# zcash/halo2

Hardware: NVIDIA H100
Metric: msm_pairs_per_s (higher is better)
Workload: dtype u32x8 (255-bit modular integers)

## Files before the change

halo2_b200/csrc/capi_msm.cu:

```cuda
#define H2_MSM_QUAD_ACCUM_REFS (g_ctx.small_accum_refs)
#include "util_kernels.cuh"
#include "msm.cuh"
#include "ipa.cuh"
#include "ntt.cuh"
#include "ecfft.cuh"
#include "fixedbase.cuh"
static_assert(H2_FB_BITS == H2_FB_BITS_CTX, "ctx.cuh: fixed_table");


static int exclusive_scan_u32(uint32_t *d, uint64_t n, cudaStream_t s, const uint32_t *only_if = nullptr) {
    const uint64_t per_block = (uint64_t)H2_SCAN_BLOCK * H2_SCAN_ITEMS;
    uint32_t nb = (uint32_t)((n + per_block - 1) / per_block);
    if (g_ctx.scan_blocks.ensure((size_t)nb * 4 + 16)) return 1;
    uint32_t *bs = g_ctx.scan_blocks.as<uint32_t>();
    LAUNCH(scan_block_sums_kernel, nb, H2_SCAN_BLOCK, 0, s, d, n, bs, only_if);
    LAUNCH(scan_single_block_kernel, 1, H2_SCAN_BLOCK, 0, s, bs, nb, only_if);
    LAUNCH(scan_apply_kernel, nb, H2_SCAN_BLOCK, 0, s, d, n, bs, only_if);
    return 0;
}

uint32_t g_chunk_cut[H2_MAX_UPLOAD_CHUNKS + 1][H2_MAX_UPLOAD_CHUNKS + 1] = {
    {0, 16, 16, 16, 16}, {0, 16, 16, 16, 16}, {0, 4, 16, 16, 16}, {0, 2, 8, 16, 16}, {0, 1, 4, 10, 16}};
static inline size_t chunk_first(size_t n, uint32_t k, uint32_t j) {
    const auto &cut = g_chunk_cut;
// ... 76 lines not shown
        FbPlan fp;
        fp.total = n; fp.sets = sets ? sets : 1u; fp.split = fb_split(n, fp.sets); fp.scalars_mont = scalars_mont ? 1u : 0u;
        record(2, H2_FB_BITS, H2_FB_WINDOWS, fp.sets, 2, 0, 0);
        const uint64_t count0 = n * fp.split;
        if (X.fb_a.ensure(fp.sets * count0 * sizeof(xyzz)) || X.fb_b.ensure(fp.sets * fb_ctas(count0, fb_fan(count0)) * sizeof(xyzz))) return 1;
        issue = [&X, fp, count0, d_scalars, d_bases, d_out, out_canonical, s]() -> int {
            auto k_acc = fb_accum_kernel<P, PS>;
            auto k_red = fb_reduce_kernel<P, PS>;
            xyzz *a = X.fb_a.as<xyzz>(), *b = X.fb_b.as<xyzz>();
            prof_begin(PROF_MSM_ACCUM0, s);
            LAUNCH(k_acc, blocks_for(fp.sets * count0, 128), 128, 0, s, fp, d_scalars, d_bases, a);
            prof_end(s);
            uint64_t count = count0, in_stride = count0;
            for (;;) {
                const uint32_t f = fb_fan(count);
                const uint64_t ctas = fb_ctas(count, f);
                LAUNCH(k_red, dim3((unsigned)ctas, fp.sets), 4 * H2_FB_QUADS, 0, s, (const xyzz *)a, count, in_stride, f, b, ctas,
                       ctas == 1 ? d_out : (jacobian *)nullptr, (uint32_t)out_canonical);
                if (ctas == 1) break;
                xyzz *t = a; a = b; b = t;
                count = ctas; in_stride = ctas;
            }
            return 0;
        };
        return msm_issue_or_replay(issue, !bc, d_scalars, d_bases, d_out, n, stride, H2_FB_BITS, fp.sets, scalars_mont, out_canonical, s);
    }
    const uint32_t glv = (!fixed && X.glv_on && n < (1ull << 30)) ? 1u : 0u;
    if (c == 0) c = X.window_override ? X.window_override : msm_default_window(n, glv);
    if (c > 24) return fail("msm: window bits > 24");
    const uint32_t K = (bc && !fixed && bc->k > 1) ? bc->k : 1u;
    const uint32_t force_cap = X.sort_bins ? 0u : H2_MSM_NO_BINS;
    MsmPlan p;
    msm_make_plan(p, n, c, 0, 0, fixed, stride, glv, sets, force_cap);
    p.chunks = K;
    p.fast = (fixed == 1 && !bc && X.fast_now && p.cap != 0) ? 1u : 0u;
    X.last_fast = p.fast != 0;
    if (p.fast && p.T < p.cap) { p.T = p.cap; p.acc_chunk[0] = p.T; }
    p.natural = (p.fast && p.G <= X.natural_max_buckets && p.max_refs <= 2 * H2_MSM_QUAD_ACCUM_REFS && (X.accum_ways <= 1 || X.accum_ways >= 12)) ? 1u : 0u;
    MsmPlan pk[H2_MAX_UPLOAD_CHUNKS];
    size_t first[H2_MAX_UPLOAD_CHUNKS + 1];
    for (uint32_t j = 0; j <= K; j++) first[j] = chunk_first(n, K, j);
    uint64_t ref_space = 0, max_items = 0, part_total = 0;
    uint32_t t_max = 0;
    for (uint32_t j = 0; j < K; j++) {
        if (K == 1) pk[0] = p;
        else msm_make_plan(pk[j], first[j + 1] - first[j], c, 0, 0, fixed, stride, glv, sets, force_cap);
        if (pk[j].ref_space >= (1ull << 32)) return fail("msm: n * windows exceeds 2^32 references");
        ref_space = pk[j].ref_space > ref_space ? pk[j].ref_space : ref_space;
        max_items = pk[j].max_items > max_items ? pk[j].max_items : max_items;
        part_total = pk[j].part_total > part_total ? pk[j].part_total : part_total;
        t_max = pk[j].T > t_max ? pk[j].T : t_max;
    }
    bool thread_per_item = false;
    for (uint32_t j = 0; j < K; j++) thread_per_item |= pk[j].max_refs > (pk[j].fixed ? 2 : 1) * H2_MSM_QUAD_ACCUM_REFS;
    record(fixed, c, p.W, p.sets, thread_per_item ? 1u : 0u, p.natural, p.fast);
    uint64_t ba_space = 0;
    if (!fixed && X.ba_rounds) {
        size_t free_b = 0, total_b = 0;
        CU(cudaMemGetInfo(&free_b, &total_b));
        for (uint32_t j = 0; j < K; j++) {
            if (pk[j].max_refs > H2_MSM_QUAD_ACCUM_REFS && (uint64_t)K * pk[j].ref_space * 56 <= free_b / 2) msm_plan_ba(pk[j], X.ba_rounds, X.ba_target);
            if (pk[j].ba) ba_space = pk[j].ref_space > ba_space ? pk[j].ref_space : ba_space;
        }
    }
    if (K == 1) p.ba = pk[0].ba;
    if (ba_space)
        for (uint32_t r = 0; r < H2_BA_MAX_ROUNDS; r++)
            if (X.ba_lv[r].ensure(K * ((ba_space >> (r + 1)) + 1) * sizeof(affine))) return 1;
    if (glv && (X.bases_phi.ensure(n * sizeof(affine)) || X.glv_parts.ensure(n * 32))) return 1;
    if (fixed && (uint64_t)p.W * stride >= (1ull << 31)) return fail("msm: window table too large for 31-bit references");
    if (p.G >= (1ull << 32) || n >= (1ull << 31)) return fail("msm: n * windows exceeds 2^32 references");
    if (scalars_mont && X.scal_canon.ensure(n * p.sets * sizeof(fe))) return 1;
    const size_t small_words = 2 * (t_max + 2) + 8;
    part_total += 1;
    if (X.counts.ensure(K * (p.G + 1) * 4) || X.cursor.ensure(K * 2 * p.G * 4) || X.refs.ensure(K * ref_space * 4) ||
        X.size_hist.ensure(K * small_words * 4) || X.items.ensure(K * max_items * sizeof(uint2)) ||
        X.bucket_sum.ensure(K * p.G * sizeof(xyzz)) || X.pkey.ensure(K * part_total * 4) || X.pstart.ensure(K * part_total * 4) ||
        X.pend.ensure(K * part_total * 4) || X.ppt.ensure(K * part_total * sizeof(xyzz)) ||
        X.ra_t.ensure((size_t)p.Wb * p.m1 * sizeof(xyzz)) || X.ra_e.ensure((size_t)p.Wb * p.m1 * sizeof(xyzz)) ||
        X.r0.ensure((size_t)p.Wb * p.nb0 * H2_R0_ROWS * sizeof(xyzz)) || X.r1.ensure((size_t)p.Wb * p.r1_rows * sizeof(xyzz)) ||
        X.wsum.ensure((size_t)p.Wb * sizeof(xyzz)))
        return 1;
    MsmBuffers Mk[H2_MAX_UPLOAD_CHUNKS];
    for (uint32_t j = 0; j < K; j++) {
        MsmBuffers &M = Mk[j];
        const size_t o = first[j];
        M.scalars = d_scalars + o; M.bases = d_bases + o; M.bases_phi = X.bases_phi.as<affine>() + o;
        M.glv_parts = X.glv_parts.as<uint32_t>() + 8 * o; M.scalars_mont = scalars_mont ? 1u : 0u;
        M.scal_canon = X.scal_canon.as<fe>() + o;
        M.counts = X.counts.as<uint32_t>() + j * (p.G + 1); M.cursor = X.cursor.as<uint32_t>() + j * 2 * p.G; M.cursor2 = M.cursor + p.G;
        M.refs = X.refs.as<uint32_t>() + j * ref_space;
        M.size_hist = X.size_hist.as<uint32_t>() + j * small_words; M.size_cursor = M.size_hist + (pk[j].T + 2); M.flags = M.size_cursor + (pk[j].T + 2);
        M.items = X.items.as<uint2>() + j * max_items;
        M.bucket_sum = X.bucket_sum.as<xyzz>() + j * p.G;
        for (uint32_t r = 0; r < H2_BA_MAX_ROUNDS; r++) M.ba[r] = ba_space ? X.ba_lv[r].as<affine>() + j * ((ba_space >> (r + 1)) + 1) : nullptr;
        M.pkey = X.pkey.as<uint32_t>() + j * part_total; M.pstart = X.pstart.as<uint32_t>() + j * part_total;
        M.pend = X.pend.as<uint32_t>() + j * part_total; M.ppt = X.ppt.as<xyzz>() + j * part_total;
        M.ra_t = X.ra_t.as<xyzz>(); M.ra_e = X.ra_e.as<xyzz>(); M.r0 = X.r0.as<xyzz>(); M.r1 = X.r1.as<xyzz>();
        M.wsum = X.wsum.as<xyzz>(); M.result = d_out;
    }
    X.last_flags = Mk[0].flags;

    {
        const uint64_t per_block = (uint64_t)H2_SCAN_BLOCK * H2_SCAN_ITEMS;
        if (X.scan_blocks.ensure((size_t)((p.G + 1 + per_block - 1) / per_block) * 4 + 16)) return 1;
    }
    issue = [&]() -> int {
        if (!p.fast) CU(cudaMemsetAsync(X.counts.p, 0, K * (p.G + 1) * 4, s));
        CU(cudaMemsetAsync(X.cursor.p, 0, K * 2 * p.G * 4, s));
        CU(cudaMemsetAsync(X.size_hist.p, 0, K * small_words * 4, s));
        CU(cudaMemsetAsync(X.bucket_sum.p, 0, K * p.G * sizeof(xyzz), s));
        if (!p.fast) CU(cudaMemsetAsync(X.pkey.p, 0xff, K * part_total * 4, s));

        auto k_bin = msm_bin_kernel<P, PS>;
        auto k_hist = msm_hist_kernel<P, PS>;
        auto k_scatter = msm_scatter_kernel<P, PS>;
        auto k_ihist = msm_item_hist_kernel<P, PS>;
        auto k_ibases = msm_item_bases_kernel<P, PS>;
        auto k_iplace = msm_item_place_kernel<P, PS>;
        auto k_accum0 = msm_accum0_kernel<P, PS>;
        auto k_accum0q = msm_accum0_quad_kernel<P, PS>;
        auto k_accum0p2 = msm_accum0_pair_kernel<P, PS>;
        auto k_accum0s2 = msm_accum0_split_kernel<P, PS, 2>;
        auto k_accum0s4 = msm_accum0_split_kernel<P, PS, 4>;
        auto k_accum0m2 = msm_accum0_multi_kernel<P, PS, 2>;
        auto k_accum0m4 = msm_accum0_multi_kernel<P, PS, 4>;
        auto k_ba = X.ba_variant == 1 ? msm_ba_round_kernel<P, PS, 4, 5> : X.ba_variant == 2 ? msm_ba_round_kernel<P, PS, 2, 4>
                  : X.ba_variant == 3 ? msm_ba_round_kernel<P, PS, 2, 5> : msm_ba_round_kernel<P, PS, 4, 4>;
        auto k_accum0p = msm_accum0_pts_kernel<P, PS>;
        auto k_accumN = msm_accumN_kernel<P, PS>;
        auto k_rest = msm_accum_rest_kernel<P, PS>;
        auto k_reduceA = msm_reduceA_kernel<P, PS>;
        auto k_r0 = msm_r0_kernel<P, PS>;
        auto k_r1 = msm_r1_kernel<P, PS>;
        auto k_wsum = msm_wsum_kernel<P, PS>;
        auto k_final = msm_final_kernel<P, PS>;
        for (uint32_t j = 0; j < K; j++) {
            const MsmPlan &q = pk[j];
            const MsmBuffers &M = Mk[j];
            if (bc && bc->k) {
                for (uint32_t e = (K > 1 ? j : 0); e < (K > 1 ? j + 1 : bc->k); e++) {
                    if (bc->wait_recorded(2 * e + 1)) return fail("msm: the upload of the inputs failed");
                    CU(cudaStreamWaitEvent(s, bc->ev_scal[e], 0));
                }
            }
            if (q.cap == 0) CU(cudaMemsetAsync(M.flags + 1, 0x01, 4, s));
            else LAUNCH(k_bin, blocks_for(q.n * q.sets, 256), 256, 0, s, q, M);
            if (!q.fast) {
                LAUNCH(k_hist, blocks_for(q.n * q.sets, 256), 256, 0, s, q, M);
                if (exclusive_scan_u32(M.counts, q.G + 1, s, M.flags + 1)) return 1;
                LAUNCH(k_scatter, blocks_for(q.n * q.sets, 256), 256, 0, s, q, M);
            }
            if (!q.natural) {
                LAUNCH(k_ihist, blocks_for(q.G, 256), 256, 0, s, q, M);
                LAUNCH(k_ibases, 1, 32, 0, s, q, M);
                LAUNCH(k_iplace, blocks_for(q.G, 256), 256, 0, s, q, M);
            }
            if (bc && bc->k) {
                for (uint32_t e = (K > 1 ? j : 0); e < (K > 1 ? j + 1 : bc->k); e++) {
                    if (bc->wait_recorded(2 * e + 2)) return fail("msm: the upload of the inputs failed");
                    CU(cudaStreamWaitEvent(s, bc->ev[e], 0));
                }
            }
            if (q.glv) {
                auto k_phi = msm_phi_kernel<P, PS>;
                LAUNCH(k_phi, blocks_for(q.n, 256), 256, 0, s, M.bases, M.bases_phi, (uint64_t)q.n);
            }
            prof_begin(PROF_MSM_ACCUM0, s);
            if (q.max_refs <= (q.fixed ? 2 : 1) * H2_MSM_QUAD_ACCUM_REFS) {
                if (X.accum_ways == 4) LAUNCH(k_accum0m4, blocks_for(q.max_items * 16, 128), 128, 0, s, q, M);
                else if (X.accum_ways == 2) LAUNCH(k_accum0m2, blocks_for(q.max_items * 8, 128), 128, 0, s, q, M);
                else if (X.accum_ways == 0) LAUNCH(k_accum0p2, blocks_for(q.max_items * 2, 128), 128, 0, s, q, M);
                else if (X.accum_ways == 12) LAUNCH(k_accum0s2, blocks_for(q.max_items * 2, 128), 128, 0, s, q, M);
                else if (X.accum_ways == 14) LAUNCH(k_accum0s4, blocks_for(q.max_items * 4, 128), 128, 0, s, q, M);
                else LAUNCH(k_accum0q, blocks_for(q.max_items * 4, 128), 128, 0, s, q, M);
            }
            else {
                for (uint32_t r = 1; r <= q.ba; r++)
                    LAUNCH(k_ba, blocks_for((q.max_items + q.ba_m[r - 1] - 1) / q.ba_m[r - 1], 128), 128, 0, s, q, M, r);
                if (q.ba) LAUNCH(k_accum0p, blocks_for(q.max_items, 128), 128, 0, s, q, M);
                LAUNCH(k_accum0, blocks_for(q.max_items, 128), 128, 0, s, q, M);
            }
            prof_end(s);
            if (!q.fast) {
                if (q.acc_levels > 1) LAUNCH(k_accumN, blocks_for(q.acc_threads[1], 128), 128, 0, s, q, M, 1u);
                if (q.acc_levels > 2) LAUNCH(k_accumN, blocks_for(q.acc_threads[2], 128), 128, 0, s, q, M, 2u);
                if (q.acc_levels > 3) LAUNCH(k_rest, 1, 256, 0, s, q, M);
            }
        }
        const MsmBuffers &M = Mk[0];
        LAUNCH(k_reduceA, blocks_for((uint64_t)p.Wb * p.m1 * 4, 128), 128, 0, s, p, M);
        LAUNCH(k_r0, blocks_for((uint64_t)p.Wb * p.nb0 * (2 + p.bits0) * 4, 128), 128, 0, s, p, M);
        LAUNCH(k_r1, p.Wb * p.r1_rows, 4 * H2_R1_QUADS, 0, s, p, M);
        LAUNCH(k_wsum, p.Wb, 128, 0, s, p, M);
        LAUNCH(k_final, 1, 64, 0, s, p, M, (uint32_t)out_canonical);
        return 0;
    };
    return msm_issue_or_replay(issue, fixed && !bc, d_scalars, d_bases, d_out, n, stride, c, sets, scalars_mont, out_canonical, s);
}

int msm_dispatch(int curve, const fe *d_scalars, int scalars_mont, const affine *d_bases, size_t n, uint32_t c,
                 jacobian *d_out, int out_canonical, cudaStream_t s, uint32_t fixed, uint64_t stride,
                 const BasesChunks *bc, uint32_t sets) {
    if (curve == H2_CURVE_PALLAS) return msm_run<FpParams, FqParams>(d_scalars, scalars_mont, d_bases, n, c, fixed, stride, d_out, out_canonical, s, bc, sets);
    if (curve == H2_CURVE_VESTA) return msm_run<FqParams, FpParams>(d_scalars, scalars_mont, d_bases, n, c, fixed, stride, d_out, out_canonical, s, bc, sets);
    return fail("unknown curve id");
}
int fixed_pass_flags(cudaStream_t s) {
    Context &X = g_ctx;
    if (!X.last_fast) return 0;
    if (!X.h_flags) CU(cudaHostAlloc((void **)&X.h_flags, 2 * sizeof(uint32_t), cudaHostAllocDefault));
    CU(cudaMemcpyAsync(X.h_flags, X.last_flags, 2 * sizeof(uint32_t), cudaMemcpyDeviceToHost, s));
    return 0;
}
bool fixed_pass_ok() {
    Context &X = g_ctx;
    return !X.last_fast || (X.h_flags[0] == 0 && X.h_flags[1] == 0);
}
static uint32_t table_window(size_t n) {
    uint32_t lg = 0;
    while ((1ull << (lg + 1)) <= n) lg++;
    uint32_t want = lg + 2;
    if (want <= 9) return 8;
    if (want <= 15) return 15;
    if (want == 16) return 15;
    if (want <= 18) return 16;
    if (want <= 20) return 17;
    return 20;
}
static int build_table(BaseSet *b, uint32_t c, cudaStream_t s) {
    if (c == 0) c = table_window(b->n);
    if (c < 4 || c > 24) return fail("window table: window bits must be in [4, 24]");
    uint32_t W = (256 + c - 1) / c;
    if ((uint64_t)W * b->n >= (1ull << 31)) return fail("window table: too many points");
    if (b->table.ensure((size_t)W * b->n * sizeof(affine))) return 1;
    if (b->curve == H2_CURVE_PALLAS) {
        auto k = msm_table_kernel<FpParams, FqParams>;
        LAUNCH(k, blocks_for(b->n, 128), 128, 0, s, b->buf.as<affine>(), b->table.as<affine>(), (uint64_t)b->n, (uint64_t)b->n, c, W);
    } else {
        auto k = msm_table_kernel<FqParams, FpParams>;
        LAUNCH(k, blocks_for(b->n, 128), 128, 0, s, b->buf.as<affine>(), b->table.as<affine>(), (uint64_t)b->n, (uint64_t)b->n, c, W);
    }
    b->c = c; b->W = W;
    return 0;
}
#define H2_FB_MAX_POINTS ((1u << 15) + 2u)
static int build_direct(BaseSet *b, cudaStream_t s) {
    if (b->n > H2_FB_MAX_POINTS) return fail("H2_BASES_DIRECT: at most 2^15 + 2 points (256 KiB of table per point)");
    if (b->c != H2_FB_BITS || b->W != H2_FB_WINDOWS) return fail("H2_BASES_DIRECT: needs the 8-bit window table");
    if (b->dtable.ensure((size_t)H2_FB_WINDOWS * H2_FB_MULTIPLES * b->n * sizeof(affine))) return 1;
    const uint64_t threads = (uint64_t)H2_FB_WINDOWS * b->n;
    if (b->curve == H2_CURVE_PALLAS) {
        auto k = fb_table_kernel<FpParams, FqParams>;
        LAUNCH(k, blocks_for(threads, 128), 128, 0, s, (const affine *)b->table.as<affine>(), b->dtable.as<affine>(), (uint64_t)b->n, (uint64_t)b->n);
    } else {
        auto k = fb_table_kernel<FqParams, FpParams>;
        LAUNCH(k, blocks_for(threads, 128), 128, 0, s, (const affine *)b->table.as<affine>(), b->dtable.as<affine>(), (uint64_t)b->n, (uint64_t)b->n);
    }
    return 0;
}
int convert_points(int curve, affine *d, size_t n, int to_mont, cudaStream_t s) {
    if (n == 0) return 0;
    if (curve == H2_CURVE_PALLAS) LAUNCH(convert_points_kernel<FpParams>, blocks_for(n, 256), 256, 0, s, d, (uint64_t)n, to_mont);
    else LAUNCH(convert_points_kernel<FqParams>, blocks_for(n, 256), 256, 0, s, d, (uint64_t)n, to_mont);
    return 0;
}

extern "C" int h2_msm_dev(int curve, const void *d_scalars, int scalars_repr, const void *d_bases, size_t n, uint32_t window_bits,
                          void *d_out_xyz, void *stream) {
    CtxLock lk;
    if (require_ready()) return 1;
    cudaStream_t s = (cudaStream_t)stream;
    if (scratch_acquire(s)) return 1;
    int rc = msm_dispatch(curve, (const fe *)d_scalars, scalars_repr == H2_REPR_MONTGOMERY, (const affine *)d_bases, n, window_bits,
                          (jacobian *)d_out_xyz, 0, s);
    if (rc) return rc;
    return scratch_release(s);
}

static int msm_host_common(int curve, const void *scalars, size_t n_scalars, const void *extra_scalar, const affine *d_bases,
                           size_t n_total, int repr, void *out_xyz, uint32_t c = 0, uint32_t fixed = 0, uint64_t stride = 0,
                           const void *host_bases = nullptr, void *d_result_peer = nullptr, int peer_dev = -1) {
    Context &X = g_ctx;
    cudaStream_t s = X.stream;
    if (scratch_acquire(s)) return 1;
    if (X.scal_in.ensure((n_total + 1) * sizeof(fe)) || X.result.ensure(sizeof(jacobian))) return 1;
    BasesChunks bc;
    std::atomic<uint32_t> recorded{0};
    std::atomic<int> up_failed{0};
    std::string up_err;
    std::thread uploader;
    if (host_bases && n_total) {
        cudaStream_t cs = X.copy_stream;
        CU(cudaEventRecord(X.ev_scalars_up, s));
        CU(cudaStreamWaitEvent(cs, X.ev_scalars_up, 0));
        bc.k = 1;
        if (n_total >= ((size_t)1 << X.chunk_min_log) && n_total >= 16 * H2_MAX_UPLOAD_CHUNKS)
            bc.k = n_total >= ((size_t)8 << X.chunk_min_log) ? H2_MAX_UPLOAD_CHUNKS : n_total >= ((size_t)2 << X.chunk_min_log) ? 3u : 2u;
        affine *db = const_cast<affine *>(d_bases);
        for (uint32_t j = 0; j < bc.k; j++) { bc.ev_scal[j] = X.ev_scal_up[j]; bc.ev[j] = X.ev_bases_up[j]; }
        bc.recorded = &recorded; bc.failed = &up_failed;
        Context *ctx = &X;
        const uint32_t k = bc.k;
        auto upload = [=, &recorded, &up_failed, &up_err]() {
            set_cur(ctx);
            auto run = [&]() -> int {
                CU(cudaSetDevice(ctx->device));
                for (uint32_t j = 0; j < k; j++) {
                    size_t lo = chunk_first(n_total, k, j), hi = chunk_first(n_total, k, j + 1);
// ... 583 lines not shown
```

halo2_b200/csrc/msm.cuh:

```cuda
#pragma once
#include "curve.cuh"
#include "glv.cuh"

namespace h2 {

H2_HD affine ld_affine(const affine *p) { affine r; r.x = fe_load(&p->x); r.y = fe_load(&p->y); return r; }
H2_HD void st_affine(affine *p, const affine &a) { fe_store(&p->x, a.x); fe_store(&p->y, a.y); }
H2_HD xyzz ld_xyzz(const xyzz *p) { xyzz r; r.x = fe_load(&p->x); r.y = fe_load(&p->y); r.zz = fe_load(&p->zz); r.zzz = fe_load(&p->zzz); return r; }
H2_HD void st_xyzz(xyzz *p, const xyzz &a) { fe_store(&p->x, a.x); fe_store(&p->y, a.y); fe_store(&p->zz, a.zz); fe_store(&p->zzz, a.zzz); }
H2_HD void st_jacobian(jacobian *p, const jacobian &a) { fe_store(&p->x, a.x); fe_store(&p->y, a.y); fe_store(&p->z, a.z); }

#define H2_MSM_INVALID_KEY 0xffffffffu
#define H2_MSM_MAX_LEVELS 12
#define H2_R0_LOG 3
#define H2_R0_ROWS 5

struct MsmPlan {
    uint64_t n;
    uint32_t c;
    uint32_t glv;
    uint32_t chunks;
    uint32_t cap;
    uint32_t cap_top;
    uint64_t g_top;
// ... 545 lines not shown
            for (uint32_t w = 1; w < W; w++) st_affine(table + (uint64_t)w * stride + i, g);
            return;
        }
        fe zs[64], pre[64];
        fe X = g.x, Y = g.y, Z = fe_one<P>(), run = fe_one<P>();
        for (uint32_t w = 1; w < W; w++) {
            for (uint32_t d = 0; d < c; d++) {
                fe A = fe_sqr<P>(X), B = fe_sqr<P>(Y), C = fe_sqr<P>(B);
                fe t = fe_add<P>(X, B);
                fe D = fe_dbl<P>(fe_sub<P>(fe_sub<P>(fe_sqr<P>(t), A), C));
                fe E = fe_add<P>(fe_dbl<P>(A), A);
                fe F = fe_sqr<P>(E);
                fe Z3 = fe_dbl<P>(fe_mul<P>(Y, Z));
                X = fe_sub<P>(fe_sub<P>(F, D), D);
                Y = fe_sub<P>(fe_mul<P>(E, fe_sub<P>(D, X)), fe_dbl<P>(fe_dbl<P>(fe_dbl<P>(C))));
                Z = Z3;
            }
            affine tmp; tmp.x = X; tmp.y = Y;
            st_affine(table + (uint64_t)w * stride + i, tmp);
            zs[w] = Z; pre[w] = run;
            run = fe_mul<P>(run, Z);
        }
        fe inv = fe_inv_gcd<P>(run);
        for (uint32_t w = W - 1; w >= 1; w--) {
            fe zi = fe_mul<P>(inv, pre[w]);
            inv = fe_mul<P>(inv, zs[w]);
            fe zi2 = fe_sqr<P>(zi);
            affine a = ld_affine(table + (uint64_t)w * stride + i);
            a.x = fe_mul<P>(a.x, zi2);
            a.y = fe_mul<P>(a.y, fe_mul<P>(zi2, zi));
            st_affine(table + (uint64_t)w * stride + i, a);
        }
    }
    static H2_HD void finish(const MsmBuffers &M, const xyzz &total, uint32_t out_canonical, uint32_t set = 0) {
        jacobian j = xyzz_to_jacobian<P>(total);
        if (out_canonical) { j.x = fe_from_mont<P>(j.x); j.y = fe_from_mont<P>(j.y); j.z = fe_from_mont<P>(j.z); }
        st_jacobian(M.result + set, j);
    }
};

#if defined(__CUDACC__)
template <bool WANT> __device__ __forceinline__ uint32_t warp_inc(uint32_t *ctr, bool active) {
    const unsigned full = 0xffffffffu;
    unsigned mask = __ballot_sync(full, active);
    if (mask == 0) return 0;
    unsigned lane = threadIdx.x & 31u;
    int first = __ffs(mask) - 1;
    unsigned long long a0 = __shfl_sync(full, (unsigned long long)ctr, first);
    bool same = !active || (unsigned long long)ctr == a0;
    if (__all_sync(full, same)) {
        uint32_t base = 0;
        if ((int)lane == first) base = atomicAdd(ctr, (uint32_t)__popc(mask));
        if (WANT) base = __shfl_sync(full, base, first);
        return base + __popc(mask & ((1u << lane) - 1u));
    }
    if (!active) return 0;
    if (WANT) return atomicAdd(ctr, 1u);
    atomicAdd(ctr, 1u);
    return 0;
}

template <class P, class PS> __global__ void __launch_bounds__(256) msm_bin_kernel(const MsmPlan p, const MsmBuffers M) {
    if (M.flags[1]) return;
    uint64_t i = (uint64_t)blockIdx.x * blockDim.x + threadIdx.x;
    bool in = i < p.n * p.sets;
    const uint64_t set = p.fixed && in ? i / p.n : 0, idx = p.fixed && in ? i % p.n : i;
    uint32_t part[2][8] = {{0, 0, 0, 0, 0, 0, 0, 0}, {0, 0, 0, 0, 0, 0, 0, 0}}, sneg[2] = {0, 0};
    const uint32_t halves = p.glv ? 2u : 1u;
    if (in) Msm<P, PS>::load_parts(p, M, i, true, part, sneg);
    bool full = false;
    for (uint32_t e = 0; e < halves; e++) {
        uint32_t carry = 0;
        for (uint32_t w0 = 0; w0 < p.W; w0 += 4) {
            uint32_t slot[4], gid[4], ref[4];
            bool act[4];
#pragma unroll
            for (int k = 0; k < 4; k++) {
                uint32_t w = w0 + k;
                int32_t d = w < p.W ? Msm<P, PS>::next_digit(part[e], w, p.c, carry) : 0;
                act[k] = in && d != 0;
                uint32_t mag = d < 0 ? (uint32_t)(-d) : (uint32_t)d;
                gid[k] = (uint32_t)((uint64_t)(p.fixed ? set : (w < p.W ? w : 0)) * p.B + (act[k] ? mag - 1 : 0));
                ref[k] = ((uint32_t)idx + (uint32_t)(p.fixed && w < p.W ? (uint64_t)w * p.stride : 0)) | (e << 30) |
                         ((((uint32_t)(d < 0)) ^ sneg[e]) << 31);
                slot[k] = warp_inc<true>(M.cursor + gid[k], act[k]);
            }
#pragma unroll
            for (int k = 0; k < 4; k++)
                if (act[k]) {
                    uint32_t lo, cap;
                    if (Msm<P, PS>::bin_of(p, gid[k], lo, cap) && slot[k] < cap) M.refs[lo + slot[k]] = ref[k];
                    else full = true;
                }
        }
    }
    if (full) M.flags[1] = 1;
}
template <class P, class PS> __global__ void __launch_bounds__(256) msm_hist_kernel(const MsmPlan p, const MsmBuffers M) {
    if (!M.flags[1]) return;
    uint64_t i = (uint64_t)blockIdx.x * blockDim.x + threadIdx.x;
    bool in = i < p.n * p.sets;
    const uint64_t set = p.fixed && in ? i / p.n : 0;
    uint32_t part[2][8] = {{0, 0, 0, 0, 0, 0, 0, 0}, {0, 0, 0, 0, 0, 0, 0, 0}}, sneg[2] = {0, 0};
    const uint32_t halves = p.glv ? 2u : 1u;
    if (in) Msm<P, PS>::load_parts(p, M, i, true, part, sneg);
    for (uint32_t e = 0; e < halves; e++) {
        uint32_t carry = 0;
        for (uint32_t w = 0; w < p.W; w++) {
            int32_t d = Msm<P, PS>::next_digit(part[e], w, p.c, carry);
            bool act = in && d != 0;
            uint32_t mag = d < 0 ? (uint32_t)(-d) : (uint32_t)d;
            uint64_t g = (uint64_t)(p.fixed ? set : w) * p.B + (act ? mag - 1 : 0);
            warp_inc<false>(M.counts + g, act);
        }
    }
}
template <class P, class PS> __global__ void __launch_bounds__(256) msm_scatter_kernel(const MsmPlan p, const MsmBuffers M) {
    if (!M.flags[1]) return;
    uint64_t i = (uint64_t)blockIdx.x * blockDim.x + threadIdx.x;
    bool in = i < p.n * p.sets;
    const uint64_t set = p.fixed && in ? i / p.n : 0, idx = p.fixed && in ? i % p.n : i;
    uint32_t part[2][8] = {{0, 0, 0, 0, 0, 0, 0, 0}, {0, 0, 0, 0, 0, 0, 0, 0}}, sneg[2] = {0, 0};
    const uint32_t halves = p.glv ? 2u : 1u;
    if (in) Msm<P, PS>::load_parts(p, M, i, false, part, sneg);
    for (uint32_t e = 0; e < halves; e++) {
        uint32_t carry = 0;
        for (uint32_t w0 = 0; w0 < p.W; w0 += 4) {
            uint32_t slot[4], gid[4], ref[4];
            bool act[4];
#pragma unroll
            for (int k = 0; k < 4; k++) {
                uint32_t w = w0 + k;
                int32_t d = w < p.W ? Msm<P, PS>::next_digit(part[e], w, p.c, carry) : 0;
                act[k] = in && d != 0;
                uint32_t mag = d < 0 ? (uint32_t)(-d) : (uint32_t)d;
                gid[k] = (uint32_t)((uint64_t)(p.fixed ? set : (w < p.W ? w : 0)) * p.B + (act[k] ? mag - 1 : 0));
                ref[k] = ((uint32_t)idx + (uint32_t)(p.fixed && w < p.W ? (uint64_t)w * p.stride : 0)) | (e << 30) |
                         ((((uint32_t)(d < 0)) ^ sneg[e]) << 31);
                slot[k] = warp_inc<true>(M.cursor2 + gid[k], act[k]);
            }
#pragma unroll
            for (int k = 0; k < 4; k++)
                if (act[k]) M.refs[M.counts[gid[k]] + slot[k]] = ref[k];
        }
    }
}
template <class P, class PS> __global__ void __launch_bounds__(256) msm_phi_kernel(const affine *bases, affine *out, uint64_t n) {
    uint64_t i = (uint64_t)blockIdx.x * blockDim.x + threadIdx.x;
    if (i >= n) return;
    affine b = ld_affine(bases + i);
    b.x = fe_mul<P>(b.x, glv_zeta<P>());
    st_affine(out + i, b);
}
template <class P, class PS> __global__ void __launch_bounds__(256) msm_item_hist_kernel(const MsmPlan p, const MsmBuffers M) {
    if (p.fast && M.flags[1]) return;
    uint64_t g = (uint64_t)blockIdx.x * blockDim.x + threadIdx.x;
    uint32_t nfull = 0, rem = 0;
    if (g < p.G) Msm<P, PS>::count_items(p, M, g, nfull, rem);
    if (nfull) atomicAdd(M.size_hist + p.T, nfull);
    warp_inc<false>(M.size_hist + rem, rem != 0);
}
template <class P, class PS> __global__ void msm_item_bases_kernel(const MsmPlan p, const MsmBuffers M) {
    if (threadIdx.x == 0 && blockIdx.x == 0) Msm<P, PS>::size_bases_body(p, M);
}
template <class P, class PS> __global__ void __launch_bounds__(256) msm_item_place_kernel(const MsmPlan p, const MsmBuffers M) {
    if (p.fast && M.flags[1]) return;
    uint64_t g = (uint64_t)blockIdx.x * blockDim.x + threadIdx.x;
    uint32_t nfull = 0, rem = 0, lo = 0;
    if (g < p.G) { Msm<P, PS>::count_items(p, M, g, nfull, rem); lo = Msm<P, PS>::bucket_lo(p, M, g); }
    if (nfull) {
        uint32_t at = atomicAdd(M.size_cursor + p.T, nfull);
        for (uint32_t k = 0; k < nfull; k++) M.items[at + k] = make_uint2((uint32_t)g, lo + k * p.T);
    }
    uint32_t at = warp_inc<true>(M.size_cursor + rem, rem != 0);
    if (rem) M.items[at] = make_uint2((uint32_t)g, lo + nfull * p.T);
}
template <class P, class PS> __global__ void __launch_bounds__(128) msm_table_kernel(const affine *bases, affine *table, uint64_t count, uint64_t stride,
                                                                                    uint32_t c, uint32_t W) {
    Msm<P, PS>::table_body(bases, table, count, stride, c, W, (uint64_t)blockIdx.x * blockDim.x + threadIdx.x);
}
template <class P, class PS> __global__ void __launch_bounds__(128, 5) msm_accum0_kernel(const MsmPlan p, const MsmBuffers M) {
    uint64_t t = (uint64_t)blockIdx.x * blockDim.x + threadIdx.x;
    Msm<P, PS>::accum0_body(p, M, t);
}
template <class P, class PS, int U, int MINB> __global__ void __launch_bounds__(128, MINB) msm_ba_round_kernel(const MsmPlan p, const MsmBuffers M, uint32_t r) {
    Msm<P, PS>::template ba_round_body<128, U>(p, M, r, (uint64_t)blockIdx.x * blockDim.x + threadIdx.x);
}
template <class P, class PS> __global__ void __launch_bounds__(128, 5) msm_accum0_pts_kernel(const MsmPlan p, const MsmBuffers M) {
    Msm<P, PS>::accum0_pts_body(p, M, (uint64_t)blockIdx.x * blockDim.x + threadIdx.x);
}
template <class P, class PS> __global__ void __launch_bounds__(128) msm_accum0_quad_kernel(const MsmPlan p, const MsmBuffers M) {
    uint64_t t = ((uint64_t)blockIdx.x * blockDim.x + threadIdx.x) >> 2;
    Msm<P, PS>::template accum0_body<QuadAdd, true>(p, M, t);
}
template <class P, class PS> __global__ void __launch_bounds__(128) msm_accum0_pair_kernel(const MsmPlan p, const MsmBuffers M) {
    uint64_t t = ((uint64_t)blockIdx.x * blockDim.x + threadIdx.x) >> 1;
    Msm<P, PS>::template accum0_body<PairAdd, true>(p, M, t);
}
template <class P, class PS, int WAYS> __global__ void __launch_bounds__(128) msm_accum0_multi_kernel(const MsmPlan p, const MsmBuffers M) {
    const uint64_t t = ((uint64_t)blockIdx.x * blockDim.x + threadIdx.x) / (4 * WAYS);
    if (p.fast && M.flags[1]) return;
    if (t >= M.size_hist[p.T + 1]) return;
    const uint32_t lane = threadIdx.x & 31u, h = (lane >> 2) & (WAYS - 1);
    const uint32_t gmask = (WAYS == 8 ? 0xffffffffu : ((1u << (4 * WAYS)) - 1u) << (lane & ~(4u * WAYS - 1u)));
    const uint2 it = M.items[t];
    const uint32_t g = it.x, start = it.y, lo = Msm<P, PS>::bucket_lo(p, M, g), hi = Msm<P, PS>::bucket_hi(p, M, g);
    const uint32_t end = start + p.T < hi ? start + p.T : hi;
    xyzz acc = xyzz_identity();
    for (uint32_t pos = start + h; pos < end; pos += WAYS) {
        const uint32_t ref = M.refs[pos];
        affine b;
        if (p.glv) b = ld_affine(((ref >> 30) & 1u ? M.bases_phi : M.bases) + (ref & 0x3fffffffu));
        else b = ld_affine(M.bases + (ref & 0x7fffffffu));
        if (ref >> 31) b.y = fe_neg<P>(b.y);
        xyzz_add_mixed_quad<P>(acc, b);
    }
#pragma unroll
    for (int step = WAYS / 2; step >= 1; step >>= 1) {
        xyzz other;
#pragma unroll
        for (int i = 0; i < 8; i++) {
            other.x.v[i] = __shfl_down_sync(gmask, acc.x.v[i], 4 * step, 4 * WAYS);
            other.y.v[i] = __shfl_down_sync(gmask, acc.y.v[i], 4 * step, 4 * WAYS);
            other.zz.v[i] = __shfl_down_sync(gmask, acc.zz.v[i], 4 * step, 4 * WAYS);
            other.zzz.v[i] = __shfl_down_sync(gmask, acc.zzz.v[i], 4 * step, 4 * WAYS);
        }
        if ((int)h < step) xyzz_add_quad<P>(acc, other);
    }
    if (h == 0) {
        typename Msm<P, PS>::Flusher F; F.M = &M; F.p = &p;
        F.flush(g, start, end, acc, p.part_offset[1] + Msm<P, PS>::item_slot(p, start, start == lo));
    }
}
template <class P, class PS, int WAYS> __global__ void __launch_bounds__(128) msm_accum0_split_kernel(const MsmPlan p, const MsmBuffers M) {
    const uint64_t t = ((uint64_t)blockIdx.x * blockDim.x + threadIdx.x) / WAYS;
    if (p.fast && M.flags[1]) return;
    const uint32_t lane = threadIdx.x & 31u, h = lane & (WAYS - 1);
    uint2 it;
    bool live = true;
    if (p.natural) {
        live = t < p.G;
        it = make_uint2((uint32_t)(live ? t : 0), live ? Msm<P, PS>::bucket_lo(p, M, live ? t : 0) : 0u);
    } else {
        live = t < M.size_hist[p.T + 1];
        it = live ? M.items[t] : make_uint2(0u, 0u);
    }
    const uint32_t g = it.x, start = it.y, lo = Msm<P, PS>::bucket_lo(p, M, g), hi = live ? Msm<P, PS>::bucket_hi(p, M, g) : start;
    const uint32_t end = start + p.T < hi ? start + p.T : hi;
    xyzz acc = xyzz_identity();
    if (start + h < end) {
        uint32_t ref = M.refs[start + h];
        affine nxt = Msm<P, PS>::ref_point(p, M, ref);
        for (uint32_t pos = start + h; pos < end; pos += WAYS) {
            affine b = nxt;
            const uint32_t neg = ref >> 31;
            if (pos + WAYS < end) { ref = M.refs[pos + WAYS]; nxt = Msm<P, PS>::ref_point(p, M, ref); }
            if (neg) b.y = fe_neg<P>(b.y);
            xyzz_add_mixed<P>(acc, b);
        }
    }
#pragma unroll
    for (int step = WAYS / 2; step >= 1; step >>= 1) {
        xyzz other;
#pragma unroll
        for (int i = 0; i < 8; i++) {
            other.x.v[i] = __shfl_down_sync(0xffffffffu, acc.x.v[i], step, WAYS);
            other.y.v[i] = __shfl_down_sync(0xffffffffu, acc.y.v[i], step, WAYS);
            other.zz.v[i] = __shfl_down_sync(0xffffffffu, acc.zz.v[i], step, WAYS);
            other.zzz.v[i] = __shfl_down_sync(0xffffffffu, acc.zzz.v[i], step, WAYS);
        }
        if ((int)h < step) xyzz_add<P>(acc, other);
    }
    if (h == 0 && live && end > start) {
        typename Msm<P, PS>::Flusher F; F.M = &M; F.p = &p;
        F.flush(g, start, end, acc, p.part_offset[1] + Msm<P, PS>::item_slot(p, start, start == lo));
    }
}
template <class P, class PS> __global__ void __launch_bounds__(128) msm_accumN_kernel(const MsmPlan p, const MsmBuffers M, uint32_t lv) {
    uint64_t t = (uint64_t)blockIdx.x * blockDim.x + threadIdx.x;
    if (t < p.acc_threads[lv]) Msm<P, PS>::accumN_body(p, M, lv, t);
}
template <class P, class PS> __global__ void __launch_bounds__(256) msm_accum_rest_kernel(const MsmPlan p, const MsmBuffers M) {
    if (!M.flags[0]) return;
    for (uint32_t lv = 3; lv < p.acc_levels; lv++) {
        for (uint64_t t = threadIdx.x; t < p.acc_threads[lv]; t += blockDim.x) Msm<P, PS>::accumN_body(p, M, lv, t);
        __threadfence();
        __syncthreads();
    }
}
template <class P, class PS> __global__ void __launch_bounds__(128) msm_reduceA_kernel(const MsmPlan p, const MsmBuffers M) {
    uint64_t t = ((uint64_t)blockIdx.x * blockDim.x + threadIdx.x) >> 2;
    Msm<P, PS>::template reduceA_body<QuadAdd>(p, M, t);
}

template <class P> __device__ __forceinline__ void block_tree_sum(xyzz *sh, xyzz &v, uint32_t row, uint32_t lane, uint32_t width) {
    st_xyzz(sh + row * width + lane, v);
    __syncthreads();
    for (uint32_t off = width >> 1; off > 0; off >>= 1) {
        if (lane < off) {
            xyzz o = ld_xyzz(sh + row * width + lane + off);
            xyzz_add<P>(v, o);
            st_xyzz(sh + row * width + lane, v);
        }
        __syncthreads();
    }
}
template <class P> __device__ __forceinline__ void quad_tree_sum(xyzz *sh, xyzz &v, uint32_t qd, uint32_t quads) {
    st_xyzz(sh + qd, v);
    __syncthreads();
    for (uint32_t off = quads >> 1; off > 0; off >>= 1) {
        if (qd < off) {
            xyzz o = ld_xyzz(sh + qd + off);
            xyzz_add_quad<P>(v, o);
            st_xyzz(sh + qd, v);
        }
        __syncthreads();
    }
}
template <class P, class PS> __global__ void __launch_bounds__(128) msm_r0_kernel(const MsmPlan p, const MsmBuffers M) {
    uint64_t tid = ((uint64_t)blockIdx.x * blockDim.x + threadIdx.x) >> 2;
    const uint32_t rows = 2 + p.bits0;
    if (tid >= (uint64_t)p.Wb * p.nb0 * rows) return;
    uint32_t row = (uint32_t)(tid % rows);
    uint64_t wb = tid / rows;
    uint32_t w = (uint32_t)(wb / p.nb0), blk = (uint32_t)(wb % p.nb0);
    xyzz v = xyzz_identity();
    const uint32_t want = row >= 2 ? 1u << (row - 2) : 0u;
    auto next_lane = [&](uint32_t l) { while (l < (1u << H2_R0_LOG) && (l & want) != want) l++; return l; };
// ... 117 lines not shown
```

Before: 232.3 million.

## Aggregate item-size histogram and placement atomics in shared memory per block

Result: faster. 235.3 million, median of 6 (+1.3%).

```diff
diff --git a/halo2_b200/csrc/capi_msm.cu b/halo2_b200/csrc/capi_msm.cu
--- a/halo2_b200/csrc/capi_msm.cu
+++ b/halo2_b200/csrc/capi_msm.cu
@@ -252,9 +252,10 @@
                 LAUNCH(k_scatter, blocks_for(q.n * q.sets, 256), 256, 0, s, q, M);
             }
             if (!q.natural) {
-                LAUNCH(k_ihist, blocks_for(q.G, 256), 256, 0, s, q, M);
+                const uint32_t per = q.G >= (1ull << 17) ? H2_ITEM_PER_THREAD : 1u;
+                LAUNCH(k_ihist, blocks_for(q.G, 256 * per), 256, 0, s, q, M, per);
                 LAUNCH(k_ibases, 1, 32, 0, s, q, M);
-                LAUNCH(k_iplace, blocks_for(q.G, 256), 256, 0, s, q, M);
+                LAUNCH(k_iplace, blocks_for(q.G, 256 * per), 256, 0, s, q, M, per);
             }
             if (bc && bc->k) {
                 for (uint32_t e = (K > 1 ? j : 0); e < (K > 1 ? j + 1 : bc->k); e++) {
diff --git a/halo2_b200/csrc/msm.cuh b/halo2_b200/csrc/msm.cuh
--- a/halo2_b200/csrc/msm.cuh
+++ b/halo2_b200/csrc/msm.cuh
@@ -721,28 +721,70 @@
     b.x = fe_mul<P>(b.x, glv_zeta<P>());
     st_affine(out + i, b);
 }
-template <class P, class PS> __global__ void __launch_bounds__(256) msm_item_hist_kernel(const MsmPlan p, const MsmBuffers M) {
+#define H2_ITEM_PER_THREAD 8
+#define H2_ITEM_SH_CLASSES 1024
+template <class P, class PS> __device__ __forceinline__ void item_sizes(const MsmPlan &p, const MsmBuffers &M, uint64_t g0, uint32_t per,
+                                                                        uint32_t (&nfull)[H2_ITEM_PER_THREAD], uint32_t (&rem)[H2_ITEM_PER_THREAD]) {
+    uint32_t cnt[H2_ITEM_PER_THREAD];
+#pragma unroll
+    for (int k = 0; k < H2_ITEM_PER_THREAD; k++) {
+        const uint64_t g = g0 + (uint64_t)k * blockDim.x;
+        cnt[k] = (uint32_t)k < per && g < p.G ? Msm<P, PS>::bucket_hi(p, M, g) - Msm<P, PS>::bucket_lo(p, M, g) : 0u;
+    }
+    bool split = false;
+#pragma unroll
+    for (int k = 0; k < H2_ITEM_PER_THREAD; k++) { nfull[k] = cnt[k] / p.T; rem[k] = cnt[k] % p.T; split |= cnt[k] > p.T; }
+    if (split) M.flags[0] = 1;
+}
+template <class P, class PS> __global__ void __launch_bounds__(256) msm_item_hist_kernel(const MsmPlan p, const MsmBuffers M, uint32_t per) {
+    __shared__ uint32_t cnt[H2_ITEM_SH_CLASSES];
     if (p.fast && M.flags[1]) return;
-    uint64_t g = (uint64_t)blockIdx.x * blockDim.x + threadIdx.x;
-    uint32_t nfull = 0, rem = 0;
-    if (g < p.G) Msm<P, PS>::count_items(p, M, g, nfull, rem);
-    if (nfull) atomicAdd(M.size_hist + p.T, nfull);
-    warp_inc<false>(M.size_hist + rem, rem != 0);
+    const uint32_t ncls = p.T + 1 < H2_ITEM_SH_CLASSES ? p.T + 1 : H2_ITEM_SH_CLASSES;
+    for (uint32_t c = threadIdx.x; c < ncls; c += blockDim.x) cnt[c] = 0;
+    uint32_t nfull[H2_ITEM_PER_THREAD], rem[H2_ITEM_PER_THREAD];
+    item_sizes<P, PS>(p, M, (uint64_t)blockIdx.x * blockDim.x * per + threadIdx.x, per, nfull, rem);
+    __syncthreads();
+#pragma unroll
+    for (int k = 0; k < H2_ITEM_PER_THREAD; k++) {
+        if (nfull[k]) atomicAdd(p.T < ncls ? cnt + p.T : M.size_hist + p.T, nfull[k]);
+        if (rem[k]) atomicAdd(rem[k] < ncls ? cnt + rem[k] : M.size_hist + rem[k], 1u);
+    }
+    __syncthreads();
+    for (uint32_t c = threadIdx.x; c < ncls; c += blockDim.x)
+        if (cnt[c]) atomicAdd(M.size_hist + c, cnt[c]);
 }
 template <class P, class PS> __global__ void msm_item_bases_kernel(const MsmPlan p, const MsmBuffers M) {
     if (threadIdx.x == 0 && blockIdx.x == 0) Msm<P, PS>::size_bases_body(p, M);
 }
-template <class P, class PS> __global__ void __launch_bounds__(256) msm_item_place_kernel(const MsmPlan p, const MsmBuffers M) {
+template <class P, class PS> __global__ void __launch_bounds__(256) msm_item_place_kernel(const MsmPlan p, const MsmBuffers M, uint32_t per) {
+    __shared__ uint32_t cnt[H2_ITEM_SH_CLASSES];
     if (p.fast && M.flags[1]) return;
-    uint64_t g = (uint64_t)blockIdx.x * blockDim.x + threadIdx.x;
-    uint32_t nfull = 0, rem = 0, lo = 0;
-    if (g < p.G) { Msm<P, PS>::count_items(p, M, g, nfull, rem); lo = Msm<P, PS>::bucket_lo(p, M, g); }
-    if (nfull) {
-        uint32_t at = atomicAdd(M.size_cursor + p.T, nfull);
-        for (uint32_t k = 0; k < nfull; k++) M.items[at + k] = make_uint2((uint32_t)g, lo + k * p.T);
-    }
-    uint32_t at = warp_inc<true>(M.size_cursor + rem, rem != 0);
-    if (rem) M.items[at] = make_uint2((uint32_t)g, lo + nfull * p.T);
+    const uint32_t ncls = p.T + 1 < H2_ITEM_SH_CLASSES ? p.T + 1 : H2_ITEM_SH_CLASSES;
+    for (uint32_t c = threadIdx.x; c < ncls; c += blockDim.x) cnt[c] = 0;
+    const uint64_t g0 = (uint64_t)blockIdx.x * blockDim.x * per + threadIdx.x;
+    uint32_t nfull[H2_ITEM_PER_THREAD], rem[H2_ITEM_PER_THREAD], at_full[H2_ITEM_PER_THREAD], at_rem[H2_ITEM_PER_THREAD];
+    item_sizes<P, PS>(p, M, g0, per, nfull, rem);
+    __syncthreads();
+#pragma unroll
+    for (int k = 0; k < H2_ITEM_PER_THREAD; k++) {
+        at_full[k] = nfull[k] ? atomicAdd(p.T < ncls ? cnt + p.T : M.size_cursor + p.T, nfull[k]) : 0u;
+        at_rem[k] = rem[k] ? atomicAdd(rem[k] < ncls ? cnt + rem[k] : M.size_cursor + rem[k], 1u) : 0u;
+    }
+    __syncthreads();
+    for (uint32_t c = threadIdx.x; c < ncls; c += blockDim.x)
+        if (cnt[c]) cnt[c] = atomicAdd(M.size_cursor + c, cnt[c]);
+    __syncthreads();
+#pragma unroll
+    for (int k = 0; k < H2_ITEM_PER_THREAD; k++) {
+        const uint64_t g = g0 + (uint64_t)k * blockDim.x;
+        if (!nfull[k] && !rem[k]) continue;
+        const uint32_t lo = Msm<P, PS>::bucket_lo(p, M, g);
+        if (nfull[k]) {
+            const uint32_t at = at_full[k] + (p.T < ncls ? cnt[p.T] : 0u);
+            for (uint32_t j = 0; j < nfull[k]; j++) M.items[at + j] = make_uint2((uint32_t)g, lo + j * p.T);
+        }
+        if (rem[k]) M.items[at_rem[k] + (rem[k] < ncls ? cnt[rem[k]] : 0u)] = make_uint2((uint32_t)g, lo + nfull[k] * p.T);
+    }
 }
 template <class P, class PS> __global__ void __launch_bounds__(128) msm_table_kernel(const affine *bases, affine *table, uint64_t count, uint64_t stride,
                                                                                     uint32_t c, uint32_t W) {
```
